# ShuoYangRobotics/Cerberus

Measured on NVIDIA H100. Metric: sliding-window solves/sec (10-frame x 150-feature windows), higher is better.
Workload: dtype f64

## Files before the change

cerberus_b200/csrc/cabi.cu:

```cuda
#include "../../include/cerberus_b200.h"
#include "solve_kernel.cuh"
#include "preint_kernel.cuh"
#include "feature_kernels.cuh"
#include "marg_kernels.cuh"
#include "pack_kernels.cuh"
#include "resident_kernels.cuh"
#include <string>
#include <vector>
#include <thread>
#include <cstring>
#include <cstdio>
#include <algorithm>
#include <chrono>
#include <cstdlib>
#include <cstdint>
#include <utility>

using namespace cerb;

static thread_local std::string g_err;
static int fail(int code, const std::string &msg) { g_err = msg; return code; }
#define CUDA_TRY(expr)                                                                                         \
    do {                                                                                                       \
        cudaError_t e_ = (expr);                                                                               \
        if (e_ != cudaSuccess) return fail(CERB_ERR_CUDA, std::string(#expr) + ": " + cudaGetErrorString(e_)); \
    } while (0)
#define COPY_TRY(h, dst, src, bytes, kind, s)                                                          \
    do {                                                                                               \
        (h)->traffic.count((kind), (bytes));                                                           \
        CUDA_TRY(cudaMemcpyAsync((dst), (src), (bytes), (kind), (s)));                                 \
    } while (0)
struct Traffic {
    int64_t h2d = 0, d2h = 0, ops = 0, staged = 0;
    void count(cudaMemcpyKind kind, size_t bytes) { if (kind == cudaMemcpyDeviceToDevice) return; (kind == cudaMemcpyHostToDevice ? h2d : d2h) += (int64_t)bytes; ops++; }
};

template <typename T> struct Resident {
    T *d = nullptr, *h = nullptr;
    size_t per = 0;
    T *at(size_t w) const { return d + w * per; }
    T *h_at(size_t w) const { return h + w * per; }
    size_t bytes(size_t n_windows) const { return n_windows * per * sizeof(T); }
};

struct CerbHandle {
    CerbSolverConfig cfg;
    int sm_count = 0, grid = 0;
    enum { MAX_CHUNKS = 32, LANES = 4 };
    cudaStream_t stream = nullptr, copy_stream = nullptr;
    cudaStream_t lane[LANES] = {};
    cudaEvent_t ev_lane[LANES] = {};
    cudaEvent_t ev_copy[MAX_CHUNKS] = {};
    cudaEvent_t ev0 = nullptr, ev1 = nullptr;
    bool ev_pending = false;
    double last_ms = 0; int last_launches = 0, last_dma_ops = 0; size_t last_staged_bytes = 0;
    int B = 0, F = 0, O = 0;
    int n = 0;
    Resident<CerbWindowDesc> rdesc; Resident<CerbFeature> rfeat; Resident<CerbObservation> robs; Resident<CerbWindowState> rstate;
    Resident<double> rpre, rlam;
    Resident<int> n_features, feat_start, feat_nobs, feat_off, flags, obs_stereo, prior_meta, rep_i, perm;
    Resident<double> obs, pre, sinfo, prior_J, prior_r, prior_x0, prior_Hp, state, state0, lam, lam0, rep_d;
    Resident<double> olam, ostate; Resident<CerbSolveReport> orep;
    double *d_ws = nullptr, *d_dbg = nullptr, *h_dbg = nullptr, *d_G = nullptr, *d_probe_repd = nullptr;
    int *d_probe_repi = nullptr;
    std::vector<void *> dev_bufs, host_bufs;
    std::vector<std::pair<uintptr_t, size_t>> regs;
    std::vector<int> nfeat, n0;
    int test_fail_factorizations = 0; double test_initial_mu = 0.0;
    bool solved = false;
    std::vector<int> h_perm; bool perm_valid = false;
    long ws_stride = 0;
    size_t smem_bytes = 0;
    std::vector<std::pair<char *, size_t>> arena; size_t arena_chunk = 0, arena_used = 0;
    Traffic traffic;
    int res_n = 0;
    Resident<int> pre_slot;
    std::vector<int> res_win;
    std::vector<int> res_extent;
    std::vector<char> res_prior_valid;
    std::vector<char> res_leg;
    Resident<double> step_J, step_r;
    bool prior_gathered = false;
    bool prior_gather_due = false;
    std::vector<unsigned char> res_mark;
};

static int create_impl(CerbHandle *h, const CerbSolverConfig *cfg, const cudaDeviceProp &prop);
#define CERB_DEVICE(h) do { if (h) { cudaError_t e_ = cudaSetDevice((h)->cfg.device); if (e_ != cudaSuccess) return fail(CERB_ERR_CUDA, std::string("cudaSetDevice: ") + cudaGetErrorString(e_)); } } while (0)

extern "C" {

const char *cerb_last_error(void) { return g_err.c_str(); }
const char *cerb_version(void) {
#if defined(CERB_CUSIM)
    return "cerberus_b200 0.1 (cusim test build)";
#else
    return "cerberus_b200 0.1 (sm_90a)";
#endif
}

void cerb_default_config(CerbSolverConfig *c) {
    std::memset(c, 0, sizeof(*c));
    c->device = 0; c->max_batch = 1024; c->max_features = 160; c->max_obs = 160 * CERB_NUM_FRAMES;
    c->max_num_iterations = 12; c->optimize_leg_bias = 1;
    c->g[0] = 0; c->g[1] = 0; c->g[2] = 9.805;
    c->visual_sqrt_info = 460.0 / 1.5; c->huber_delta = 1.0;
    c->initial_trust_region_radius = 1e4; c->max_trust_region_radius = 1e16; c->min_trust_region_radius = 1e-32;
    c->min_relative_decrease = 1e-3; c->function_tolerance = 1e-6; c->gradient_tolerance = 1e-10; c->parameter_tolerance = 1e-8;
}

void cerb_default_preint_config(CerbPreintConfig *p) {
    std::memset(p, 0, sizeof(*p));
    p->acc_n = 0.9; p->acc_n_z = 2.5; p->gyr_n = 0.05; p->acc_w = 0.0004; p->gyr_w = 0.0002;
    p->phi_n = 1e-5; p->dphi_n = 1e-5; p->rho_c_n = 1e-8; p->rho_nc_n = 1e-11;
    p->v_n_min_xy = 1e-3; p->v_n_min_z = 5e-3; p->v_n_min = 5e-3; p->v_n_max = 900.0;
    p->v_n_force_thres_ratio = 0.8; p->v_n_term1_steep = 10; p->v_n_term2_var_rescale = 1e-6; p->v_n_term3_distance_rescale = 1e-3;
    p->contact_sensor_type = 0;
    const double ox[4] = {0.1805, 0.1805, -0.1805, -0.1805}, oy[4] = {0.047, -0.047, 0.047, -0.047}, d[4] = {0.0838, -0.0838, 0.0838, -0.0838};
    for (int l = 0; l < 4; l++) { p->rho_fix[l][0] = ox[l]; p->rho_fix[l][1] = oy[l]; p->rho_fix[l][2] = d[l]; p->rho_fix[l][3] = 0.21; }
    p->R_br[0] = p->R_br[4] = p->R_br[8] = 1.0;
}


int cerb_create(const CerbSolverConfig *cfg, CerbHandle **out) {
    if (!cfg || !out) return fail(CERB_ERR_BAD_ARGUMENT, "cerb_create: null argument");
    if (cfg->max_batch < 1 || cfg->max_features < 1 || cfg->max_features > CERB_MAX_FEATURES || cfg->max_obs < 1)
        return fail(CERB_ERR_BAD_ARGUMENT, "cerb_create: bad capacities");
    int ndev = 0;
    if (cudaGetDeviceCount(&ndev) != cudaSuccess || ndev <= cfg->device)
        return fail(CERB_ERR_NO_DEVICE, "cerb_create: no CUDA device (this library has no CPU fallback)");
    CUDA_TRY(cudaSetDevice(cfg->device));
    cudaDeviceProp prop;
    CUDA_TRY(cudaGetDeviceProperties(&prop, cfg->device));
    CerbHandle *h = new CerbHandle();
    const int rc = create_impl(h, cfg, prop);
    if (rc != CERB_OK) { const std::string keep = g_err; cerb_destroy(h); g_err = keep; return rc; }
    *out = h;
    return CERB_OK;
}

}

template <typename T> static cudaError_t dmalloc(CerbHandle *h, T **p, size_t n) {
    const cudaError_t e = cudaMalloc((void **)p, n * sizeof(T));
    if (e == cudaSuccess) h->dev_bufs.push_back(*p);
    return e;
}
template <typename T> static cudaError_t hmalloc(CerbHandle *h, T **p, size_t n) {
    const cudaError_t e = cudaMallocHost((void **)p, n * sizeof(T));
    if (e == cudaSuccess) h->host_bufs.push_back(*p);
    return e;
}
template <typename T> static cudaError_t alloc(CerbHandle *h, Resident<T> &a, size_t per, bool mirror = false) {
    a.per = per;
    const cudaError_t e = dmalloc(h, &a.d, (size_t)h->B * per);
    return (e != cudaSuccess || !mirror) ? e : hmalloc(h, &a.h, (size_t)h->B * per);
}

static int create_impl(CerbHandle *h, const CerbSolverConfig *cfg, const cudaDeviceProp &prop) {
    h->cfg = *cfg; h->sm_count = prop.multiProcessorCount;
    if (const char *e = std::getenv("CERB_TEST_FAIL_FACTORIZATIONS")) h->test_fail_factorizations = std::atoi(e);
    if (const char *e = std::getenv("CERB_TEST_INITIAL_MU")) h->test_initial_mu = std::atof(e);
    h->B = cfg->max_batch; h->F = cfg->max_features; h->O = cfg->max_obs;
    h->grid = std::min(h->B, h->sm_count);
    h->smem_bytes = (size_t)SMEM_DOUBLES * sizeof(double);
    if (h->smem_bytes > prop.sharedMemPerBlockOptin) return fail(CERB_ERR_CUDA, "solve kernel needs more shared memory than the device offers");
    CUDA_TRY(cudaFuncSetAttribute(vilo_solve_kernel, cudaFuncAttributeMaxDynamicSharedMemorySize, (int)h->smem_bytes));
    CUDA_TRY(cudaFuncSetAttribute(prior_prepare_kernel, cudaFuncAttributeMaxDynamicSharedMemorySize, (int)(PRIOR_TROWS * PRIOR_TLD * sizeof(double))));
    CUDA_TRY(cudaStreamCreate(&h->stream));
    CUDA_TRY(cudaStreamCreate(&h->copy_stream));
    h->lane[0] = h->stream;
    for (int k = 1; k < CerbHandle::LANES; k++) CUDA_TRY(cudaStreamCreate(&h->lane[k]));
    for (int k = 0; k < CerbHandle::LANES; k++) CUDA_TRY(cudaEventCreate(&h->ev_lane[k]));
    for (int k = 0; k < CerbHandle::MAX_CHUNKS; k++) CUDA_TRY(cudaEventCreate(&h->ev_copy[k]));
    CUDA_TRY(cudaEventCreate(&h->ev0)); CUDA_TRY(cudaEventCreate(&h->ev1));
    const size_t F = h->F, O = h->O;
    h->ws_stride = ws_size(h->F);
    CUDA_TRY(alloc(h, h->rdesc, 1, true)); CUDA_TRY(alloc(h, h->rfeat, F, true)); CUDA_TRY(alloc(h, h->robs, O, true)); CUDA_TRY(alloc(h, h->rstate, 1, true));
    CUDA_TRY(alloc(h, h->rpre, CERB_WINDOW_SIZE * RAW_PRE_STRIDE, true)); CUDA_TRY(alloc(h, h->rlam, F, true)); CUDA_TRY(alloc(h, h->perm, F));
    CUDA_TRY(alloc(h, h->olam, F, true)); CUDA_TRY(alloc(h, h->ostate, ST_STRIDE, true)); CUDA_TRY(alloc(h, h->orep, 1, true));
    CUDA_TRY(alloc(h, h->n_features, 1)); CUDA_TRY(alloc(h, h->feat_start, F)); CUDA_TRY(alloc(h, h->feat_nobs, F)); CUDA_TRY(alloc(h, h->feat_off, F));
    CUDA_TRY(alloc(h, h->flags, 1)); CUDA_TRY(alloc(h, h->obs_stereo, O)); CUDA_TRY(alloc(h, h->prior_meta, PRIOR_META_STRIDE)); CUDA_TRY(alloc(h, h->rep_i, 4));
    CUDA_TRY(alloc(h, h->obs, NOBS_PLANES * O)); CUDA_TRY(alloc(h, h->pre, CERB_WINDOW_SIZE * PRE_STRIDE)); CUDA_TRY(alloc(h, h->sinfo, CERB_WINDOW_SIZE * 961));
    CUDA_TRY(alloc(h, h->prior_J, PRIOR_LD * PRIOR_LD, true)); CUDA_TRY(alloc(h, h->prior_r, PRIOR_LD, true)); CUDA_TRY(alloc(h, h->prior_x0, CERB_MAX_PRIOR_BLOCKS * 9));
    CUDA_TRY(alloc(h, h->prior_Hp, PRIOR_LD * PRIOR_LD));
    CUDA_TRY(alloc(h, h->state, ST_STRIDE)); CUDA_TRY(alloc(h, h->state0, ST_STRIDE)); CUDA_TRY(alloc(h, h->lam, F)); CUDA_TRY(alloc(h, h->lam0, F)); CUDA_TRY(alloc(h, h->rep_d, 2));
    CUDA_TRY(dmalloc(h, &h->d_ws, (size_t)CerbHandle::LANES * h->grid * h->ws_stride)); CUDA_TRY(dmalloc(h, &h->d_dbg, 2 * (NR + F) + 8)); CUDA_TRY(dmalloc(h, &h->d_G, 4));
    CUDA_TRY(dmalloc(h, &h->d_probe_repi, 4)); CUDA_TRY(dmalloc(h, &h->d_probe_repd, 2)); CUDA_TRY(hmalloc(h, &h->h_dbg, 2 * (NR + F) + 8));
    CUDA_TRY(alloc(h, h->pre_slot, CERB_WINDOW_SIZE + 1, true));
    h->nfeat.assign(h->B, 0); h->n0.assign(h->B, 0); h->res_extent.assign(h->B, 0); h->res_prior_valid.assign(h->B, 0); h->res_leg.assign(h->B, 1);
    CUDA_TRY(cudaMemcpy(h->d_G, cfg->g, 3 * sizeof(double), cudaMemcpyHostToDevice));
    return CERB_OK;
}

extern "C" {

void cerb_destroy(CerbHandle *h) {
    if (!h) return;
    cudaSetDevice(h->cfg.device);
    if (h->stream) cudaStreamSynchronize(h->stream);
    for (void *p : h->dev_bufs) cudaFree(p);
    for (auto &c : h->arena) cudaFree(c.first);
    for (auto &r : h->regs) cudaHostUnregister((void *)r.first);
    for (void *p : h->host_bufs) cudaFreeHost(p);
    if (h->ev0) cudaEventDestroy(h->ev0);
    if (h->ev1) cudaEventDestroy(h->ev1);
    for (int k = 0; k < CerbHandle::MAX_CHUNKS; k++) if (h->ev_copy[k]) cudaEventDestroy(h->ev_copy[k]);
    for (int k = 0; k < CerbHandle::LANES; k++) if (h->ev_lane[k]) cudaEventDestroy(h->ev_lane[k]);
    for (int k = 1; k < CerbHandle::LANES; k++) if (h->lane[k]) cudaStreamDestroy(h->lane[k]);
    if (h->copy_stream) cudaStreamDestroy(h->copy_stream);
    if (h->stream) cudaStreamDestroy(h->stream);
    delete h;
}

}
// ... 138 lines not shown
    plan_rows(h, pl, w0, cn, h->prior_J, 0, 1, 0,
              [&](int w) { return (const void *)descs[w].prior.linearized_jacobians; }, [&](int w) { return descs[w].prior.valid ? (size_t)descs[w].prior.n * descs[w].prior.n * 8 : (size_t)0; });
    plan_rows(h, pl, w0, cn, h->prior_r, 0, 1, 0,
              [&](int w) { return (const void *)descs[w].prior.linearized_residuals; }, [&](int w) { return descs[w].prior.valid ? (size_t)descs[w].prior.n * 8 : (size_t)0; });
    return run_plan(h, pl, s, t_stage_ms);
}

static int enqueue_pack(CerbHandle *h, int w0, int cn, cudaStream_t s) {
    PackParams P;
    P.n = cn; P.maxF = h->F; P.maxObs = h->O;
    P.rdesc = h->rdesc.at(w0); P.rfeat = h->rfeat.at(w0); P.robs = h->robs.at(w0); P.rpre = h->rpre.at(w0); P.rstate = h->rstate.at(w0); P.rlam = h->rlam.at(w0);
    P.n_features = h->n_features.at(w0); P.feat_start = h->feat_start.at(w0); P.feat_nobs = h->feat_nobs.at(w0); P.feat_off = h->feat_off.at(w0); P.flags = h->flags.at(w0);
    P.obs_stereo = h->obs_stereo.at(w0); P.prior_meta = h->prior_meta.at(w0); P.perm = h->perm.at(w0);
    P.obs = h->obs.at(w0); P.pre = h->pre.at(w0); P.prior_x0 = h->prior_x0.at(w0); P.state0 = h->state0.at(w0); P.lam0 = h->lam0.at(w0);
    if (h->res_n) { P.pre_slot = h->pre_slot.d; P.window = h->pre_slot.d + (size_t)cn * CERB_WINDOW_SIZE; }
    CERB_LAUNCH(pack_kernel, std::min(cn, 8 * h->sm_count), PACK_THREADS, 0, s, P);
    CUDA_TRY(cudaGetLastError());
    return CERB_OK;
}
static int upload(CerbHandle *h, int n, const CerbWindowDesc *descs, const CerbWindowState *states) {
    h->last_dma_ops = 0; h->last_staged_bytes = 0;
    int rc = upload_raw(h, 0, n, descs, states, h->stream, nullptr); if (rc) return rc;
    rc = enqueue_pack(h, 0, n, h->stream); if (rc) return rc;
    h->n = n; h->solved = false; h->perm_valid = false;
    return CERB_OK;
}
static int ensure_perm(CerbHandle *h) {
    if (h->perm_valid) return CERB_OK;
    h->h_perm.resize((size_t)h->B * h->perm.per);
    CUDA_TRY(cudaMemcpyAsync(h->h_perm.data(), h->perm.d, h->perm.bytes(h->n), cudaMemcpyDeviceToHost, h->stream));
    CUDA_TRY(cudaStreamSynchronize(h->stream));
    h->perm_valid = true;
    return CERB_OK;
}

static const Resident<double> &batch_prior_J(const CerbHandle *h) { return h->prior_gathered ? h->step_J : h->prior_J; }
static const Resident<double> &batch_prior_r(const CerbHandle *h) { return h->prior_gathered ? h->step_r : h->prior_r; }

static SolveParams make_params(CerbHandle *h, int w0, int n, int max_iters, double *dbg, int dbg_window) {
    SolveParams P;
    std::memset(&P, 0, sizeof(P));
    const CerbSolverConfig &c = h->cfg;
    P.n_windows = n; P.maxF = h->F; P.maxObs = h->O; P.max_iters = max_iters; P.optimize_leg_bias = c.optimize_leg_bias;
    for (int k = 0; k < 3; k++) P.G[k] = c.g[k];
    P.sqrt_info = c.visual_sqrt_info; P.huber = c.huber_delta;
    P.radius0 = c.initial_trust_region_radius; P.max_radius = c.max_trust_region_radius; P.min_radius = c.min_trust_region_radius;
    P.min_rel_dec = c.min_relative_decrease; P.ftol = c.function_tolerance; P.gtol = c.gradient_tolerance; P.ptol = c.parameter_tolerance;
    P.n_features = h->n_features.at(w0); P.feat_start = h->feat_start.at(w0); P.feat_nobs = h->feat_nobs.at(w0); P.feat_off = h->feat_off.at(w0); P.flags = h->flags.at(w0);
    P.obs = h->obs.at(w0); P.obs_stereo = h->obs_stereo.at(w0); P.pre = h->pre.at(w0); P.sinfo = h->sinfo.at(w0);
    P.prior_J = batch_prior_J(h).at(w0); P.prior_r = batch_prior_r(h).at(w0); P.prior_x0 = h->prior_x0.at(w0); P.prior_Hp = h->prior_Hp.at(w0); P.prior_meta = h->prior_meta.at(w0);
    P.state = h->state.at(w0); P.lam = h->lam.at(w0); P.rep_i = h->rep_i.at(w0); P.rep_d = h->rep_d.at(w0); P.ws = h->d_ws; P.ws_stride = h->ws_stride;
    P.dbg = dbg; P.dbg_window = dbg_window;
    P.test_fail_factorizations = h->test_fail_factorizations; P.test_initial_mu = h->test_initial_mu;
    P.no_bulk_copy = std::getenv("CERB_NO_TMA") != nullptr;
    return P;
}

static void enqueue_prepare(CerbHandle *h, int w0, int n, cudaStream_t s) {
    const int nfac = n * CERB_WINDOW_SIZE;
    CERB_LAUNCH(imu_leg_prepare_kernel, (nfac + 1) / 2, 64, 0, s, nfac, (const double *)h->pre.at(w0), h->sinfo.at(w0));
    CERB_LAUNCH(prior_prepare_kernel, n, 256, (size_t)PRIOR_TROWS * PRIOR_TLD * sizeof(double), s, (const double *)batch_prior_J(h).at(w0), (const int *)h->prior_meta.at(w0), h->prior_Hp.at(w0));
}

static int gather_priors(CerbHandle *h, cudaStream_t s) {
    if (!h->prior_gather_due) return CERB_OK;
    const int n = h->n;
    CERB_LAUNCH(prior_gather_kernel, std::min(n, 8 * h->sm_count), 256, 0, s, n, (const int *)(h->pre_slot.d + (size_t)n * CERB_WINDOW_SIZE), (const CerbWindowDesc *)h->rdesc.d,
                (const double *)h->prior_J.d, (const double *)h->prior_r.d, h->step_J.d, h->step_r.d);
    CUDA_TRY(cudaGetLastError());
    h->prior_gather_due = false;
    return CERB_OK;
}

static int enqueue_solve(CerbHandle *h, int w0, int n, int max_iters, double *dbg, int dbg_window, bool restore = true, bool probe = false, int lane = 0) {
    cudaStream_t s = h->lane[lane];
    if (restore) {
        CUDA_TRY(cudaMemcpyAsync(h->state.at(w0), h->state0.at(w0), h->state.bytes(n), cudaMemcpyDeviceToDevice, s));
        CUDA_TRY(cudaMemcpyAsync(h->lam.at(w0), h->lam0.at(w0), h->lam.bytes(n), cudaMemcpyDeviceToDevice, s));
    }
    int rc = gather_priors(h, s); if (rc) return rc;
    enqueue_prepare(h, w0, n, s);
    SolveParams P = make_params(h, w0, n, max_iters, dbg, dbg_window);
    P.ws = h->d_ws + (size_t)lane * h->grid * h->ws_stride;
    if (probe) { P.rep_i = h->d_probe_repi; P.rep_d = h->d_probe_repd; }
    if (max_iters > 0) h->solved = true;
    CERB_LAUNCH(vilo_solve_kernel, std::min(n, h->grid), SOLVE_THREADS, h->smem_bytes, s, P);
    CUDA_TRY(cudaGetLastError());
    return CERB_OK;
}
static int launch_solve(CerbHandle *h, int max_iters, double *dbg, int dbg_window, bool timed) {
    const int n = h->n;
    if (n < 1) return fail(CERB_ERR_BAD_ARGUMENT, "no resident batch");
    if (timed) CUDA_TRY(cudaEventRecord(h->ev0, h->stream));
    int rc = enqueue_solve(h, 0, n, max_iters, dbg, dbg_window); if (rc) return rc;
    if (timed) { CUDA_TRY(cudaEventRecord(h->ev1, h->stream)); h->ev_pending = true; h->last_launches = 3; }
    return CERB_OK;
}

static int collect_time(CerbHandle *h) {
    if (h->ev_pending) {
        CUDA_TRY(cudaEventSynchronize(h->ev1));
        float ms = 0; CUDA_TRY(cudaEventElapsedTime(&ms, h->ev0, h->ev1));
        h->last_ms = ms; h->ev_pending = false;
    }
    return CERB_OK;
}
// ... 712 lines not shown
```

cerberus_b200/csrc/solve_kernel.cuh:

```cuda
#pragma once
#include "eval_kernels.cuh"

namespace cerb {

#if defined(CERB_PHASE_TIMING) && !defined(CERB_CUSIM)
__device__ unsigned long long g_phase_cycles[48];
#define PH_DECL() long long ph_t = clock64()
#define PH_MARK_T(id, t) do { if ((threadIdx.x & 31) == 0) { const long long ph_n = clock64(); if (threadIdx.x == (t)) atomicAdd(&g_phase_cycles[id], (unsigned long long)(ph_n - ph_t)); ph_t = ph_n; } __syncwarp(); } while (0)
#define PH_MARK(id) PH_MARK_T(id, 0)
#define PH_ARG , long long &ph_t
#define PH_FWD , ph_t
#else
#define PH_DECL()
#define PH_MARK_T(id, t)
#define PH_MARK(id)
#define PH_ARG
#define PH_FWD
#endif

enum { CERB_WINDOW = 10, NX = 79, NYB = 13, NFR = 11, NY = 143, NR = 222, NRP = 224, HXX_SZ = 79 * 79, HXY_SZ = 79 * 143, X_TD = 78, SOLVE_THREADS = 256, FT = 64, TILE_LD = 33, NOBS_PLANES = 9 };
enum { HBLK = NYB * NYB, AD_SZ = NFR * HBLK, BO_SZ = (NFR - 1) * HBLK };
#ifndef CERB_SOLVE_MIN_BLOCKS
#define CERB_SOLVE_MIN_BLOCKS 1
#endif
enum { PIMG_HXY = HXX_SZ + 1, PIMG_REST = HXY_SZ + AD_SZ + BO_SZ, PIMG_SZ = PIMG_HXY + PIMG_REST, SMEM_HXX_PAD = 3 };
static_assert((PIMG_HXY * 8) % 16 == 0 && (PIMG_REST * 8) % 16 == 0 && ((HXX_SZ + SMEM_HXX_PAD) * 8) % 16 == 0, "bulk-copy alignment of the prior image");

struct SolveParams {
    int n_windows, maxF, maxObs, max_iters, optimize_leg_bias;
    double G[3], sqrt_info, huber;
    double radius0, max_radius, min_radius, min_rel_dec, ftol, gtol, ptol;
    const int *n_features, *feat_start, *feat_nobs, *feat_off, *flags;
    const double *obs; const int *obs_stereo;
    const double *pre;
    const double *sinfo;
    const double *prior_J, *prior_r, *prior_x0, *prior_Hp; const int *prior_meta;
    double *state, *lam;
    int *rep_i; double *rep_d;
    double *ws;
    long ws_stride;
    double *dbg; int dbg_window;
    double test_initial_mu;
    int no_bulk_copy;
    int test_fail_factorizations;
};

CERB_HD long ws_vecs(int F) { return (long)NX * F; }
CERB_HD long ws_prior(int F) { return (long)NX * F + 9L * F; }
CERB_HD long ws_chunks(int F) { return ws_prior(F) + PIMG_SZ; }
CERB_HD long ws_imuplan(int F) { return (ws_chunks(F) + (F + 4) / 2 + 8 + 1) & ~1L; }
CERB_HD long ws_size(int F) { return ws_imuplan(F) + 15 * 2 * 32 * 4 / 2 + 8; }
struct CtaWs {
    double *W, *hh, *gl, *sl, *Dl, *ghl, *gnl, *stl, *lamc, *sinv;
    int *chunks;
    int *imu_plan;
    double *pimg;
    int F;
};
CERB_D CtaWs ws_carve(const SolveParams &P) {
    double *ws = P.ws + (size_t)blockIdx.x * P.ws_stride;
    const int F = P.maxF;
    CtaWs v;
    v.W = ws;
    v.hh = ws + ws_vecs(F); v.gl = v.hh + F; v.sl = v.gl + F; v.Dl = v.sl + F; v.ghl = v.Dl + F; v.gnl = v.ghl + F; v.stl = v.gnl + F; v.lamc = v.stl + F; v.sinv = v.lamc + F;
    v.chunks = reinterpret_cast<int *>(ws + ws_chunks(F)); v.imu_plan = reinterpret_cast<int *>(ws + ws_imuplan(F));
    v.pimg = ws + ws_prior(F); v.F = F;
    return v;
}

struct Smem {
    double *Hxx, *Hxy, *Ad, *Bo;
    double *g, *sc, *D, *gh, *gn, *stp, *yv;
    double *xs, *xc;
    double *Rw, *Rex;
    double *Ju;
    double *lin;
    double *pdx, *pr;
    double *red;
    double *wj;
    double *sca;
    double *chain_col;
    double *idg;
    double *idx;
    int *ti;
    unsigned long long *mbar;
    double *tile;
};
enum { S_RADIUS = 0, S_MU, S_REUSE, S_XCOST, S_CCOST, S_ALPHA, S_GNORM2, S_GNNORM2, S_GDOTGN, S_MODEL, S_STEPNORM, S_XNORM, S_DLNORM,
       S_OK, S_DONE, S_TERM, S_ITER, S_NSUCC, S_INVALID, S_GMAX, S_INIT_COST, S_P, S_Q, S_VHV, S_LCOST, S_LNORM, S_LGMAX, S_COUNT };
static_assert(S_COUNT <= 32, "scalar slots overlap the chain's column line");
enum { TI_PRIOR_MAP = 0, TI_NCHUNKS = 96, TI_CHUNK_CACHE = 97, TI_CACHED_CHUNKS = 15, TI_CHAIN_DONE = 130, TI_IMU_MASK = 131, TI_INTS = 132 };
static_assert(TI_PRIOR_MAP + CERB_MAX_PRIOR_DIM <= TI_NCHUNKS && TI_CHUNK_CACHE + 2 * TI_CACHED_CHUNKS <= TI_CHAIN_DONE && TI_IMU_MASK < TI_INTS && TI_INTS % 2 == 0,
              "s.ti slots overlap");
enum { SMEM_DOUBLES = HXX_SZ + SMEM_HXX_PAD + HXY_SZ + AD_SZ + BO_SZ + 7 * NRP + 2 * ST_STRIDE + 99 + 18 + 3 + 31 * 39 + 960 + 192 + 8 * 256 + 128 * 8 + 32 + 32 + TI_INTS / 2 + 144 + 80 };

CERB_D void smem_carve(double *base, Smem &s) {
    double *p = base;
// ... 101 lines not shown
    if (g == 0) return c < 6 ? 6 * a + c : (c == 6 ? X_TD : -2);
    if (c >= 6) return -1;
    return g == 1 ? 6 * j + c : (g == 2 ? 66 + c : 72 + c);
}
CERB_D void vis_scatter(Smem &s, int ga, int gb, int ra, int rb, int a, int j, double v) {
    if (ga == gb && ra > rb) return;
    const int da = vis_col_dest(ga, ra, a, j), db = vis_col_dest(gb, rb, a, j);
    if (da == -1 || db == -1) return;
    if (da == -2) { if (db >= 0) s.g[db] += v; return; }
    if (db == -2) { s.g[da] += v; return; }
    if (da <= db) s.Hxx[da * NX + db] += v; else s.Hxx[db * NX + da] += v;
}
CERB_D void vis_jplan(const Smem &s, const double *smem_base, int el, int *base, int *ca, int *cj) {
    const int blk = el >> 6, ra = (el >> 3) & 7, rb = el & 7;
    const int hxx = (int)(s.Hxx - smem_base), g = (int)(s.g - smem_base);
    *base = -1; *ca = 0; *cj = 0;
    if (rb >= 6) return;
    if (blk == 0) {
        if (ra < 6) { *base = hxx + ra * NX + rb; *ca = 6 * NX; *cj = 6; }
        else if (ra == 6) { *base = hxx + rb * NX + X_TD; *cj = 6 * NX; }
        else { *base = g + rb; *cj = 6; }
    } else {
        if (ra >= 6 || (blk == 1 && ra > rb)) return;
        *base = hxx + ra * NX + (blk == 1 ? rb : (blk == 2 ? 66 + rb : 72 + rb)); *cj = 6 * NX + (blk == 1 ? 6 : 0);
    }
}
CERB_NOINLINE double vision_linearize(const SolveParams &P, int w, const double *x, const double *lam, double *W, double *hh, double *gl,
                                      const double *sl, bool prescale, const int *chunks, int tid) {
    CERB_DYN_SMEM(double, smem_base);
    Smem s; smem_carve(smem_base, s);
    const int nF = P.n_features[w], F = P.maxF, mo = P.maxObs;
    const double *obs = P.obs + (size_t)w * NOBS_PLANES * P.maxObs;
    const int *stereo = P.obs_stereo + (size_t)w * P.maxObs;
    double cost = 0.0;
    PH_DECL();
    for (int i = tid; i < NX * nF; i += SOLVE_THREADS) W[(i / nF) * F + (i % nF)] = 0.0;
    __syncthreads();
    const int wid = tid >> 5, lane = tid & 31;
    const int cam = tid >> 7, jj = (tid >> 6) & 1, fl = tid & 63;
    double *T = s.tile;
    double *jp = s.Ju;
    double *pp = (wid < 5) ? s.Ju + 8 * VJ_SZ + VP_SZ * wid : s.tile + VT_SZ + VP_SZ * (wid - 5);
    const int c8 = lane >> 2;
    const double *tq[4];
    bool tv[4];
    for (int g = 0; g < 4; g++) { const int pc = g == 0 ? c8 : 8 + 6 * (g - 1) + c8; tv[g] = (g == 0) || c8 < 6; tq[g] = T + (tv[g] ? pc : 0) * VT_LD + (lane & 3); }
    int jbase, jca, jcj;
    vis_jplan(s, smem_base, tid, &jbase, &jca, &jcj);
    const int nchunks = s.ti[TI_NCHUNKS];
    for (int ch = 0; ch < nchunks; ch++) {
        int c0, nc, a;
        if (ch < TI_CACHED_CHUNKS) { const int *cc = s.ti + TI_CHUNK_CACHE + 2 * ch; c0 = cc[0]; nc = cc[1] >> 8; a = cc[1] & 255; }
        else { c0 = chunks[1 + ch]; nc = chunks[2 + ch] - c0; a = P.feat_start[(size_t)w * F + c0]; }
        const int f = c0 + fl;
        const bool ev = fl < nc;
        int nobs = 0, off = 0;
        double lamf = 1.0, pix = 0.0, piy = 0.0, vix = 0.0, viy = 0.0, tdi = 0.0;
        const double slf = (prescale && ev) ? sl[f] : 1.0;
        if (ev) {
            nobs = P.feat_nobs[(size_t)w * F + f]; off = P.feat_off[(size_t)w * F + f];
            lamf = 1.0 / lam[f];
            pix = obs[0 * mo + off]; piy = obs[1 * mo + off]; vix = obs[2 * mo + off]; viy = obs[3 * mo + off]; tdi = obs[8 * mo + off];
        }
        ObsVals ov; ov.px = ov.py = ov.vx = ov.vy = ov.td = 0.0; ov.stereo = 0;
        { const int j = a + jj; if (ev && j < a + nobs) obs_fetch(obs, stereo, mo, off + (j - a), cam, ov); }
        for (int k = lane; k < VP_SZ; k += 32) pp[k] = 0.0;
        if (tid < 2 * (NFR - 1 - a)) {
            const int jq = a + 1 + (tid >> 1), cq = tid & 1;
            const m33 Rc = ldm33(cq ? s.Rex + 9 : s.Rex);
            const m33 A = mulT33(Rc, tr33(ldm33(s.Rw + 9 * jq)));
            const m33 ARi = mul33(A, ldm33(s.Rw + 9 * a));
            const m33 Tm = mul33(ARi, ldm33(s.Rex));
            double *C = s.lin + 27 * tid;
            for (int k = 0; k < 9; k++) { C[k] = A.m[k]; C[9 + k] = ARi.m[k]; C[18 + k] = Tm.m[k]; }
        } else if (tid == 32) {
            const m33 T3 = mul33(tr33(ldm33(s.Rex + 9)), ldm33(s.Rex));
            for (int k = 0; k < 9; k++) s.lin[540 + k] = T3.m[k];
        }
        __syncthreads();
        double h = 0.0, gq = 0.0, wT = 0.0, wI[6], wE0[6], wE1[6];
        for (int k = 0; k < 6; k++) { wI[k] = 0.0; wE0[k] = 0.0; wE1[k] = 0.0; }
        PH_MARK(20);
        for (int j0 = a; j0 < NFR; j0 += 2) {
            const int j = j0 + jj;
            bool valid = ev && j < a + nobs;
            int kind = PROJ_K1;
            if (valid) {
                if (j == a) { if (cam == 0 || !ov.stereo) valid = false; kind = PROJ_K3; }
                else if (cam == 1) { if (!ov.stereo) valid = false; kind = PROJ_K2; }
            }
            double wjv[6] = {0, 0, 0, 0, 0, 0};
            double *t0 = T + tid, *t1 = T + 256 + tid;
            if (valid) {
                const d3 tic = ld3(x + ST_EX), tc = kind == PROJ_K1 ? tic : ld3(x + ST_EX + 7);
                const double *Rcp = kind == PROJ_K1 ? s.Rex : s.Rex + 9;
                const double tdv = x[ST_TD];
                const d3 pts_i = mk3(pix, piy, 1.0), vel_i = mk3(vix, viy, 0.0);
                const d3 pts_i_td = pts_i - (tdv - tdi) * vel_i;
                const double pjx_td = ov.px - (tdv - ov.td) * ov.vx, pjy_td = ov.py - (tdv - ov.td) * ov.vy;
                const double inv_l = lamf;
                const d3 p_ci = inv_l * pts_i_td;
                const d3 p_bi = mv33(ldm33(s.Rex), p_ci) + tic;
                d3 p_bj = p_bi;
                if (kind != PROJ_K3) p_bj = mTv33(ldm33(s.Rw + 9 * j), (mv33(ldm33(s.Rw + 9 * a), p_bi) + ld3(x + ST_POSE + 7 * a)) - ld3(x + ST_POSE + 7 * j));
                const d3 p_cj = mTv33(ldm33(Rcp), p_bj - tc);
                const double iz = 1.0 / p_cj.z;
                double r0 = P.sqrt_info * (p_cj.x * iz - pjx_td), r1 = P.sqrt_info * (p_cj.y * iz - pjy_td);
                double cf; const double hw = huber_weight(P.huber, r0 * r0 + r1 * r1, &cf);
                cost += cf;
                r0 *= hw; r1 *= hw;
                const double q = hw * P.sqrt_info * iz, c0 = -q * p_cj.x * iz, c1 = -q * p_cj.y * iz;
                const d3 e0 = mk3(q, 0.0, c0), e1 = mk3(0.0, q, c1);
#define VIS_U(M, u0, u1) const d3 u0 = mk3(q * (M)[0] + c0 * (M)[6], q * (M)[1] + c0 * (M)[7], q * (M)[2] + c0 * (M)[8]), u1 = mk3(q * (M)[3] + c1 * (M)[6], q * (M)[4] + c1 * (M)[7], q * (M)[5] + c1 * (M)[8])
#define VIS_PUT(col, a0, a1) do { t0[(col) * VT_LD] = (a0); t1[(col) * VT_LD] = (a1); } while (0)
#define VIS_PUT3(col, v0_, v1_) do { VIS_PUT(col, (v0_).x, (v1_).x); VIS_PUT((col) + 1, (v0_).y, (v1_).y); VIS_PUT((col) + 2, (v0_).z, (v1_).z); } while (0)
                const double *Tm = kind == PROJ_K3 ? s.lin + 540 : s.lin + 27 * (2 * (j - a - 1) + cam) + 18;
                VIS_U(Tm, uT0, uT1);
                const d3 ptl = kind == PROJ_K3 ? pts_i : pts_i_td;
                const double l0 = -inv_l * inv_l * dot3(uT0, ptl), l1 = -inv_l * inv_l * dot3(uT1, ptl);
                const double d0 = -inv_l * dot3(uT0, vel_i) + hw * P.sqrt_info * ov.vx, d1 = -inv_l * dot3(uT1, vel_i) + hw * P.sqrt_info * ov.vy;
                h += l0 * l0 + l1 * l1; gq += l0 * r0 + l1 * r1; wT += d0 * l0 + d1 * l1;
                VIS_PUT(6, d0, d1); VIS_PUT(7, r0, r1);
                const d3 uC0 = mk3(q * Rcp[0] + c0 * Rcp[2], q * Rcp[3] + c0 * Rcp[5], q * Rcp[6] + c0 * Rcp[8]);
                const d3 uC1 = mk3(q * Rcp[1] + c1 * Rcp[2], q * Rcp[4] + c1 * Rcp[5], q * Rcp[7] + c1 * Rcp[8]);
                const d3 er0 = cross3(e0, p_cj), er1 = cross3(e1, p_cj);
                const d3 et0 = cross3(p_ci, uT0), et1 = cross3(p_ci, uT1);
                d3 E0t0, E0t1, E0r0, E0r1, E1t0, E1t1, E1r0, E1r1;
                if (kind == PROJ_K3) {
                    for (int k = 0; k < 6; k++) { VIS_PUT(k, 0.0, 0.0); VIS_PUT(8 + k, 0.0, 0.0); }
                    E0t0 = uC0; E0t1 = uC1; E0r0 = et0; E0r1 = et1; E1t0 = -uC0; E1t1 = -uC1; E1r0 = er0; E1r1 = er1;
                } else {
                    const double *C = s.lin + 27 * (2 * (j - a - 1) + cam);
                    VIS_U(C, uA0, uA1);
                    VIS_U(C + 9, uR0, uR1);
                    const d3 ir0 = cross3(p_bi, uR0), ir1 = cross3(p_bi, uR1);
                    const d3 jr0 = cross3(uC0, p_bj), jr1 = cross3(uC1, p_bj);
                    VIS_PUT3(0, uA0, uA1); VIS_PUT3(3, ir0, ir1);
                    VIS_PUT3(8, -uA0, -uA1); VIS_PUT3(11, jr0, jr1);
                    wI[0] += uA0.x * l0 + uA1.x * l1; wI[1] += uA0.y * l0 + uA1.y * l1; wI[2] += uA0.z * l0 + uA1.z * l1;
                    wI[3] += ir0.x * l0 + ir1.x * l1; wI[4] += ir0.y * l0 + ir1.y * l1; wI[5] += ir0.z * l0 + ir1.z * l1;
                    wjv[0] = -(uA0.x * l0 + uA1.x * l1); wjv[1] = -(uA0.y * l0 + uA1.y * l1); wjv[2] = -(uA0.z * l0 + uA1.z * l1);
                    wjv[3] = jr0.x * l0 + jr1.x * l1; wjv[4] = jr0.y * l0 + jr1.y * l1; wjv[5] = jr0.z * l0 + jr1.z * l1;
                    if (kind == PROJ_K1) {
                        E0t0 = uR0 - uC0; E0t1 = uR1 - uC1; E0r0 = et0 + er0; E0r1 = et1 + er1;
                        E1t0 = mk3(0, 0, 0); E1t1 = E1t0; E1r0 = E1t0; E1r1 = E1t0;
                    } else {
                        E0t0 = uR0; E0t1 = uR1; E0r0 = et0; E0r1 = et1; E1t0 = -uC0; E1t1 = -uC1; E1r0 = er0; E1r1 = er1;
                    }
                }
                VIS_PUT3(14, E0t0, E0t1); VIS_PUT3(17, E0r0, E0r1); VIS_PUT3(20, E1t0, E1t1); VIS_PUT3(23, E1r0, E1r1);
                wE0[0] += E0t0.x * l0 + E0t1.x * l1; wE0[1] += E0t0.y * l0 + E0t1.y * l1; wE0[2] += E0t0.z * l0 + E0t1.z * l1;
                wE0[3] += E0r0.x * l0 + E0r1.x * l1; wE0[4] += E0r0.y * l0 + E0r1.y * l1; wE0[5] += E0r0.z * l0 + E0r1.z * l1;
                wE1[0] += E1t0.x * l0 + E1t1.x * l1; wE1[1] += E1t0.y * l0 + E1t1.y * l1; wE1[2] += E1t0.z * l0 + E1t1.z * l1;
                wE1[3] += E1r0.x * l0 + E1r1.x * l1; wE1[4] += E1r0.y * l0 + E1r1.y * l1; wE1[5] += E1r0.z * l0 + E1r1.z * l1;
#undef VIS_U
#undef VIS_PUT
#undef VIS_PUT3
            } else {
                for (int k = 0; k < VT_COLS; k++) { t0[k * VT_LD] = 0.0; t1[k * VT_LD] = 0.0; }
            }
            const bool wrow = valid && j != a;
            if (wrow && cam == 0) for (int k = 0; k < 6; k++) W[(size_t)(6 * j + k) * F + f] = wjv[k] * (prescale ? s.sc[6 * j + k] * slf : 1.0);
            __syncthreads();
            PH_MARK(21);
            double wprev[6] = {0, 0, 0, 0, 0, 0};
            if (wrow && cam == 1) for (int k = 0; k < 6; k++) wprev[k] = W[(size_t)(6 * j + k) * F + f];
            { const int jn = j + 2; ov.stereo = 0; if (ev && jn < a + nobs) obs_fetch(obs, stereo, mo, off + (jn - a), cam, ov); }
            {
                const int jw = j0 + (wid >> 2), hw = (wid >> 1) & 1, par = wid & 1;
                const bool k3 = (jw == a);
                const int nkt = (nc + 3) >> 2;
                const bool work = jw < NFR && par < nkt;
                double acc[10][2];
                for (int k = 0; k < 10; k++) { acc[k][0] = 0.0; acc[k][1] = 0.0; }
                if (work) {
                    const int rb0 = 256 * hw + 64 * (wid >> 2) + 4 * par;
                    if (!k3) {
                        double v0 = tq[0][rb0], v1 = tv[1] ? tq[1][rb0] : 0.0, v2 = tv[2] ? tq[2][rb0] : 0.0;
                        for (int ks = par; ks < nkt; ks += 2) {
                            const int rn = rb0 + 4 * (ks + 2 - par);
                            const bool more = ks + 2 < nkt;
                            const double n0 = more ? tq[0][rn] : 0.0, n1 = (more && tv[1]) ? tq[1][rn] : 0.0, n2 = (more && tv[2]) ? tq[2][rn] : 0.0;
                            CERB_DMMA(acc[0][0], acc[0][1], v0, v0, acc[0][0], acc[0][1]);
                            CERB_DMMA(acc[1][0], acc[1][1], v0, v1, acc[1][0], acc[1][1]);
                            CERB_DMMA(acc[2][0], acc[2][1], v0, v2, acc[2][0], acc[2][1]);
                            CERB_DMMA(acc[4][0], acc[4][1], v1, v1, acc[4][0], acc[4][1]);
                            CERB_DMMA(acc[5][0], acc[5][1], v1, v2, acc[5][0], acc[5][1]);
                            CERB_DMMA(acc[7][0], acc[7][1], v2, v2, acc[7][0], acc[7][1]);
                            v0 = n0; v1 = n1; v2 = n2;
                        }
                    }
                    {
                        const int rb1 = rb0 + 128;
                        double v0 = tq[0][rb1], v1 = (!k3 && tv[1]) ? tq[1][rb1] : 0.0, v2 = tv[2] ? tq[2][rb1] : 0.0, v3 = tv[3] ? tq[3][rb1] : 0.0;
                        for (int ks = par; ks < nkt; ks += 2) {
                            const int rn = rb1 + 4 * (ks + 2 - par);
                            const bool more = ks + 2 < nkt;
                            const double n0 = more ? tq[0][rn] : 0.0, n1 = (more && !k3 && tv[1]) ? tq[1][rn] : 0.0, n2 = (more && tv[2]) ? tq[2][rn] : 0.0, n3 = (more && tv[3]) ? tq[3][rn] : 0.0;
                            CERB_DMMA(acc[0][0], acc[0][1], v0, v0, acc[0][0], acc[0][1]);
                            CERB_DMMA(acc[2][0], acc[2][1], v0, v2, acc[2][0], acc[2][1]);
                            CERB_DMMA(acc[3][0], acc[3][1], v0, v3, acc[3][0], acc[3][1]);
                            CERB_DMMA(acc[7][0], acc[7][1], v2, v2, acc[7][0], acc[7][1]);
                            CERB_DMMA(acc[8][0], acc[8][1], v2, v3, acc[8][0], acc[8][1]);
                            CERB_DMMA(acc[9][0], acc[9][1], v3, v3, acc[9][0], acc[9][1]);
                            if (!k3) {
                                CERB_DMMA(acc[1][0], acc[1][1], v0, v1, acc[1][0], acc[1][1]);
                                CERB_DMMA(acc[4][0], acc[4][1], v1, v1, acc[4][0], acc[4][1]);
                                CERB_DMMA(acc[5][0], acc[5][1], v1, v2, acc[5][0], acc[5][1]);
                                CERB_DMMA(acc[6][0], acc[6][1], v1, v3, acc[6][0], acc[6][1]);
                            }
                            v0 = n0; v1 = n1; v2 = n2; v3 = n3;
                        }
                    }
                    PH_MARK(28);
                    const int o = (lane >> 2) * 8 + 2 * (lane & 3);
                    pp[0 * 64 + o] += acc[0][0]; pp[0 * 64 + o + 1] += acc[0][1];
                    pp[1 * 64 + o] += acc[2][0]; pp[1 * 64 + o + 1] += acc[2][1];
                    pp[2 * 64 + o] += acc[3][0]; pp[2 * 64 + o + 1] += acc[3][1];
                    pp[3 * 64 + o] += acc[7][0]; pp[3 * 64 + o + 1] += acc[7][1];
                    pp[4 * 64 + o] += acc[8][0]; pp[4 * 64 + o + 1] += acc[8][1];
                    pp[5 * 64 + o] += acc[9][0]; pp[5 * 64 + o + 1] += acc[9][1];
                }
                {
                    const int o = wid * VJ_SZ + (lane >> 2) * 8 + 2 * (lane & 3);
                    jp[o] = acc[1][0]; jp[o + 1] = acc[1][1];
                    jp[64 + o] = acc[4][0]; jp[64 + o + 1] = acc[4][1];
                    jp[128 + o] = acc[5][0]; jp[128 + o + 1] = acc[5][1];
                    jp[192 + o] = acc[6][0]; jp[192 + o + 1] = acc[6][1];
                }
            }
            if (wrow && cam == 1) for (int k = 0; k < 6; k++) W[(size_t)(6 * j + k) * F + f] = wprev[k] + wjv[k] * (prescale ? s.sc[6 * j + k] * slf : 1.0);
            PH_MARK(29);
            __syncthreads();
            PH_MARK(22);
            if (jbase >= 0) {
                _Pragma("unroll")
                for (int fj = 0; fj < 2; fj++) {
                    const int jf = j0 + fj;
                    if (jf >= NFR || jf == a) continue;
                    const double *q = jp + (4 * fj) * VJ_SZ + tid;
                    smem_base[jbase + jca * a + jcj * jf] += ((q[0] + q[VJ_SZ]) + q[2 * VJ_SZ]) + q[3 * VJ_SZ];
                }
            }
            PH_MARK(23);
        }
        __syncthreads();
        {
            double *ex = T;
            ex[0 * 256 + tid] = h; ex[1 * 256 + tid] = gq; ex[2 * 256 + tid] = wT;
            for (int k = 0; k < 6; k++) { ex[(3 + k) * 256 + tid] = wI[k]; ex[(9 + k) * 256 + tid] = wE0[k]; ex[(15 + k) * 256 + tid] = wE1[k]; }
        }
        __syncthreads();
        for (int e = tid; e < VP_SZ; e += SOLVE_THREADS) {
            double v = 0.0;
            for (int wq = 0; wq < 8; wq++) v += ((wq < 5) ? s.Ju + 8 * VJ_SZ + VP_SZ * wq : s.tile + VT_SZ + VP_SZ * (wq - 5))[e];
            const int blk = e >> 6, ra = (e >> 3) & 7, rb = e & 7;
            const int ga = blk < 3 ? 0 : (blk < 5 ? 2 : 3), gb = blk == 0 ? 0 : (blk == 1 || blk == 3 ? 2 : 3);
            vis_scatter(s, ga, gb, ra, rb, a, a, v);
        }
        if (tid < 64 && ev) {
            const double *ex = T;
            double q[21];
            for (int k = 0; k < 21; k++) q[k] = ((ex[k * 256 + tid] + ex[k * 256 + 64 + tid]) + ex[k * 256 + 128 + tid]) + ex[k * 256 + 192 + tid];
            hh[f] = q[0] * slf * slf; gl[f] = q[1] * slf;
            W[(size_t)X_TD * F + f] = q[2] * (prescale ? s.sc[X_TD] * slf : 1.0);
            for (int k = 0; k < 6; k++) {
                W[(size_t)(6 * a + k) * F + f] = q[3 + k] * (prescale ? s.sc[6 * a + k] * slf : 1.0);
                W[(size_t)(66 + k) * F + f] = q[9 + k] * (prescale ? s.sc[66 + k] * slf : 1.0);
                W[(size_t)(72 + k) * F + f] = q[15 + k] * (prescale ? s.sc[72 + k] * slf : 1.0);
            }
        }
        __syncthreads();
        PH_MARK(24);
    }
    return cost;
}

CERB_D void imu_lin_all(const SolveParams &P, Smem &s, int w, const double *x, bool want_jac, int tid) {
    if (tid < CERB_WINDOW) {
        const double *pre = P.pre + ((size_t)w * CERB_WINDOW + tid) * PRE_STRIDE;
        IMULegLin *L = reinterpret_cast<IMULegLin *>(s.lin + 96 * tid);
        imu_leg_linearize(pre, x + ST_POSE + 7 * tid, x + ST_SB + 9 * tid, x + ST_LB + 4 * tid, x + ST_POSE + 7 * (tid + 1),
                          x + ST_SB + 9 * (tid + 1), x + ST_LB + 4 * (tid + 1), P.G, want_jac, L);
    }
    __syncthreads();
}

CERB_D double prior_residual(const SolveParams &P, Smem &s, int w, const double *x, int tid) {
    const int *meta = P.prior_meta + (size_t)w * PRIOR_META_STRIDE;
    if (!meta[0]) return 0.0;
    const int n = meta[1], nb = meta[2];
    const double *J = P.prior_J + (size_t)w * PRIOR_LD * PRIOR_LD, *r0 = P.prior_r + (size_t)w * PRIOR_LD, *x0 = P.prior_x0 + (size_t)w * 16 * 9;
    if (tid < nb) {
        const int kind = meta[4 + 3 * tid], index = meta[5 + 3 * tid], col = meta[6 + 3 * tid];
        prior_block_dx(kind, x + prior_block_state_offset(kind, index), x0 + 9 * tid, s.pdx + col);
    }
    __syncthreads();
    int parts = SOLVE_THREADS / n; if (parts > 4) parts = 4; if (parts < 1) parts = 1;
    const int kc = (n + parts - 1) / parts;
    double *part = s.red;
    for (int e = tid; e < parts * n; e += SOLVE_THREADS) {
        const int p = e / n, i = e % n;
        const int k1 = (p + 1) * kc < n ? (p + 1) * kc : n;
        double t = 0.0;
        for (int k = p * kc; k < k1; k++) t += J[(size_t)k * n + i] * s.pdx[k];
        part[p * PRIOR_LD + i] = t;
    }
    __syncthreads();
    double cost = 0.0;
    for (int i = tid; i < n; i += SOLVE_THREADS) {
        double t = r0[i];
        for (int p = 0; p < parts; p++) t += part[p * PRIOR_LD + i];
        s.pr[i] = t; cost += 0.5 * t * t;
// ... 1181 lines not shown
```

Baseline: 34820.

## Process four frames per pass for small feature chunks in visual linearization

When a feature chunk holds at most 32 features, threads with lane index 32 and above now handle frames offset by two. Each outer-loop pass therefore covers four observing frames instead of two, which roughly halves the number of passes and barriers for small chunks. The upper-half partial sums (cost, Hessian, gradient, W rows) are exchanged through shared memory and folded into the lower half, and the DMMA block reductions run twice per pass. The cost is extra syncthreads, added shared-memory traffic, and register pressure from keeping the acc array live outside its block. An environment flag restores the old two-frame path.

```diff
diff --git a/cerberus_b200/csrc/cabi.cu b/cerberus_b200/csrc/cabi.cu
--- a/cerberus_b200/csrc/cabi.cu
+++ b/cerberus_b200/csrc/cabi.cu
@@ -67,6 +67,7 @@
     std::vector<std::pair<uintptr_t, size_t>> regs;
     std::vector<int> nfeat, n0;
     int test_fail_factorizations = 0; double test_initial_mu = 0.0;
+    int test_two_frame_passes = 0;
     bool solved = false;
     std::vector<int> h_perm; bool perm_valid = false;
     long ws_stride = 0;
@@ -161,6 +162,7 @@
     h->cfg = *cfg; h->sm_count = prop.multiProcessorCount;
     if (const char *e = std::getenv("CERB_TEST_FAIL_FACTORIZATIONS")) h->test_fail_factorizations = std::atoi(e);
     if (const char *e = std::getenv("CERB_TEST_INITIAL_MU")) h->test_initial_mu = std::atof(e);
+    if (const char *e = std::getenv("CERB_TEST_TWO_FRAME_PASSES")) h->test_two_frame_passes = std::atoi(e) != 0;
     h->B = cfg->max_batch; h->F = cfg->max_features; h->O = cfg->max_obs;
     h->grid = std::min(h->B, h->sm_count);
     h->smem_bytes = (size_t)SMEM_DOUBLES * sizeof(double);
@@ -405,6 +407,7 @@
     P.state = h->state.at(w0); P.lam = h->lam.at(w0); P.rep_i = h->rep_i.at(w0); P.rep_d = h->rep_d.at(w0); P.ws = h->d_ws; P.ws_stride = h->ws_stride;
     P.dbg = dbg; P.dbg_window = dbg_window;
     P.test_fail_factorizations = h->test_fail_factorizations; P.test_initial_mu = h->test_initial_mu;
+    P.test_two_frame_passes = h->test_two_frame_passes;
     P.no_bulk_copy = std::getenv("CERB_NO_TMA") != nullptr;
     return P;
 }
diff --git a/cerberus_b200/csrc/solve_kernel.cuh b/cerberus_b200/csrc/solve_kernel.cuh
--- a/cerberus_b200/csrc/solve_kernel.cuh
+++ b/cerberus_b200/csrc/solve_kernel.cuh
@@ -43,6 +43,7 @@
     double test_initial_mu;
     int no_bulk_copy;
     int test_fail_factorizations;
+    int test_two_frame_passes;
 };
 
 CERB_HD long ws_vecs(int F) { return (long)NX * F; }
@@ -250,8 +251,11 @@
         int c0, nc, a;
         if (ch < TI_CACHED_CHUNKS) { const int *cc = s.ti + TI_CHUNK_CACHE + 2 * ch; c0 = cc[0]; nc = cc[1] >> 8; a = cc[1] & 255; }
         else { c0 = chunks[1 + ch]; nc = chunks[2 + ch] - c0; a = P.feat_start[(size_t)w * F + c0]; }
-        const int f = c0 + fl;
-        const bool ev = fl < nc;
+        const int fp = (nc <= 32 && !P.test_two_frame_passes) ? 4 : 2;
+        const bool up = fp == 4 && fl >= 32;
+        const int fe = up ? fl - 32 : fl, jo = up ? 2 : 0;
+        const int f = c0 + fe;
+        const bool ev = fe < nc;
         int nobs = 0, off = 0;
         double lamf = 1.0, pix = 0.0, piy = 0.0, vix = 0.0, viy = 0.0, tdi = 0.0;
         const double slf = (prescale && ev) ? sl[f] : 1.0;
@@ -261,7 +265,7 @@
             pix = obs[0 * mo + off]; piy = obs[1 * mo + off]; vix = obs[2 * mo + off]; viy = obs[3 * mo + off]; tdi = obs[8 * mo + off];
         }
         ObsVals ov; ov.px = ov.py = ov.vx = ov.vy = ov.td = 0.0; ov.stereo = 0;
-        { const int j = a + jj; if (ev && j < a + nobs) obs_fetch(obs, stereo, mo, off + (j - a), cam, ov); }
+        { const int j = a + jj + jo; if (ev && j < a + nobs) obs_fetch(obs, stereo, mo, off + (j - a), cam, ov); }
         for (int k = lane; k < VP_SZ; k += 32) pp[k] = 0.0;
         if (tid < 2 * (NFR - 1 - a)) {
             const int jq = a + 1 + (tid >> 1), cq = tid & 1;
@@ -278,9 +282,11 @@
         __syncthreads();
         double h = 0.0, gq = 0.0, wT = 0.0, wI[6], wE0[6], wE1[6];
         for (int k = 0; k < 6; k++) { wI[k] = 0.0; wE0[k] = 0.0; wE1[k] = 0.0; }
+        double *cfu = s.Ju + 8 * VJ_SZ + 5 * VP_SZ + (tid >> 6) * 32 + (tid & 31);
+        if (up) *cfu = 0.0;
         PH_MARK(20);
-        for (int j0 = a; j0 < NFR; j0 += 2) {
-            const int j = j0 + jj;
+        for (int j0 = a; j0 < NFR; j0 += fp) {
+            const int j = j0 + jj + jo;
             bool valid = ev && j < a + nobs;
             int kind = PROJ_K1;
             if (valid) {
@@ -305,7 +311,7 @@
                 const double iz = 1.0 / p_cj.z;
                 double r0 = P.sqrt_info * (p_cj.x * iz - pjx_td), r1 = P.sqrt_info * (p_cj.y * iz - pjy_td);
                 double cf; const double hw = huber_weight(P.huber, r0 * r0 + r1 * r1, &cf);
-                cost += cf;
+                if (up) *cfu = cf; else cost += cf;
                 r0 *= hw; r1 *= hw;
                 const double q = hw * P.sqrt_info * iz, c0 = -q * p_cj.x * iz, c1 = -q * p_cj.y * iz;
                 const d3 e0 = mk3(q, 0.0, c0), e1 = mk3(0.0, q, c1);
@@ -363,82 +369,111 @@
             PH_MARK(21);
             double wprev[6] = {0, 0, 0, 0, 0, 0};
             if (wrow && cam == 1) for (int k = 0; k < 6; k++) wprev[k] = W[(size_t)(6 * j + k) * F + f];
-            { const int jn = j + 2; ov.stereo = 0; if (ev && jn < a + nobs) obs_fetch(obs, stereo, mo, off + (jn - a), cam, ov); }
+            { const int jn = j + fp; ov.stereo = 0; if (ev && jn < a + nobs) obs_fetch(obs, stereo, mo, off + (jn - a), cam, ov); }
+            double acc[10][2];
             {
-                const int jw = j0 + (wid >> 2), hw = (wid >> 1) & 1, par = wid & 1;
-                const bool k3 = (jw == a);
+                const int hw = (wid >> 1) & 1, par = wid & 1;
                 const int nkt = (nc + 3) >> 2;
-                const bool work = jw < NFR && par < nkt;
-                double acc[10][2];
-                for (int k = 0; k < 10; k++) { acc[k][0] = 0.0; acc[k][1] = 0.0; }
-                if (work) {
-                    const int rb0 = 256 * hw + 64 * (wid >> 2) + 4 * par;
-                    if (!k3) {
-                        double v0 = tq[0][rb0], v1 = tv[1] ? tq[1][rb0] : 0.0, v2 = tv[2] ? tq[2][rb0] : 0.0;
-                        for (int ks = par; ks < nkt; ks += 2) {
-                            const int rn = rb0 + 4 * (ks + 2 - par);
-                            const bool more = ks + 2 < nkt;
-                            const double n0 = more ? tq[0][rn] : 0.0, n1 = (more && tv[1]) ? tq[1][rn] : 0.0, n2 = (more && tv[2]) ? tq[2][rn] : 0.0;
-                            CERB_DMMA(acc[0][0], acc[0][1], v0, v0, acc[0][0], acc[0][1]);
-                            CERB_DMMA(acc[1][0], acc[1][1], v0, v1, acc[1][0], acc[1][1]);
-                            CERB_DMMA(acc[2][0], acc[2][1], v0, v2, acc[2][0], acc[2][1]);
-                            CERB_DMMA(acc[4][0], acc[4][1], v1, v1, acc[4][0], acc[4][1]);
-                            CERB_DMMA(acc[5][0], acc[5][1], v1, v2, acc[5][0], acc[5][1]);
-                            CERB_DMMA(acc[7][0], acc[7][1], v2, v2, acc[7][0], acc[7][1]);
-                            v0 = n0; v1 = n1; v2 = n2;
-                        }
-                    }
-                    {
-                        const int rb1 = rb0 + 128;
-                        double v0 = tq[0][rb1], v1 = (!k3 && tv[1]) ? tq[1][rb1] : 0.0, v2 = tv[2] ? tq[2][rb1] : 0.0, v3 = tv[3] ? tq[3][rb1] : 0.0;
-                        for (int ks = par; ks < nkt; ks += 2) {
-                            const int rn = rb1 + 4 * (ks + 2 - par);
-                            const bool more = ks + 2 < nkt;
-                            const double n0 = more ? tq[0][rn] : 0.0, n1 = (more && !k3 && tv[1]) ? tq[1][rn] : 0.0, n2 = (more && tv[2]) ? tq[2][rn] : 0.0, n3 = (more && tv[3]) ? tq[3][rn] : 0.0;
-                            CERB_DMMA(acc[0][0], acc[0][1], v0, v0, acc[0][0], acc[0][1]);
-                            CERB_DMMA(acc[2][0], acc[2][1], v0, v2, acc[2][0], acc[2][1]);
-                            CERB_DMMA(acc[3][0], acc[3][1], v0, v3, acc[3][0], acc[3][1]);
-                            CERB_DMMA(acc[7][0], acc[7][1], v2, v2, acc[7][0], acc[7][1]);
-                            CERB_DMMA(acc[8][0], acc[8][1], v2, v3, acc[8][0], acc[8][1]);
-                            CERB_DMMA(acc[9][0], acc[9][1], v3, v3, acc[9][0], acc[9][1]);
-                            if (!k3) {
+                _Pragma("unroll 1")
+                for (int u = 0; u < fp / 2; u++) {
+                    const int jw = j0 + (wid >> 2) + 2 * u;
+                    const bool k3 = (jw == a);
+                    const bool work = jw < NFR && par < nkt;
+                    for (int k = 0; k < 10; k++) { acc[k][0] = 0.0; acc[k][1] = 0.0; }
+                    if (work) {
+                        const int rb0 = 256 * hw + 64 * (wid >> 2) + 32 * u + 4 * par;
+                        if (!k3) {
+                            double v0 = tq[0][rb0], v1 = tv[1] ? tq[1][rb0] : 0.0, v2 = tv[2] ? tq[2][rb0] : 0.0;
+                            for (int ks = par; ks < nkt; ks += 2) {
+                                const int rn = rb0 + 4 * (ks + 2 - par);
+                                const bool more = ks + 2 < nkt;
+                                const double n0 = more ? tq[0][rn] : 0.0, n1 = (more && tv[1]) ? tq[1][rn] : 0.0, n2 = (more && tv[2]) ? tq[2][rn] : 0.0;
+                                CERB_DMMA(acc[0][0], acc[0][1], v0, v0, acc[0][0], acc[0][1]);
                                 CERB_DMMA(acc[1][0], acc[1][1], v0, v1, acc[1][0], acc[1][1]);
+                                CERB_DMMA(acc[2][0], acc[2][1], v0, v2, acc[2][0], acc[2][1]);
                                 CERB_DMMA(acc[4][0], acc[4][1], v1, v1, acc[4][0], acc[4][1]);
                                 CERB_DMMA(acc[5][0], acc[5][1], v1, v2, acc[5][0], acc[5][1]);
-                                CERB_DMMA(acc[6][0], acc[6][1], v1, v3, acc[6][0], acc[6][1]);
+                                CERB_DMMA(acc[7][0], acc[7][1], v2, v2, acc[7][0], acc[7][1]);
+                                v0 = n0; v1 = n1; v2 = n2;
                             }
-                            v0 = n0; v1 = n1; v2 = n2; v3 = n3;
                         }
+                        {
+                            const int rb1 = rb0 + 128;
+                            double v0 = tq[0][rb1], v1 = (!k3 && tv[1]) ? tq[1][rb1] : 0.0, v2 = tv[2] ? tq[2][rb1] : 0.0, v3 = tv[3] ? tq[3][rb1] : 0.0;
+                            for (int ks = par; ks < nkt; ks += 2) {
+                                const int rn = rb1 + 4 * (ks + 2 - par);
+                                const bool more = ks + 2 < nkt;
+                                const double n0 = more ? tq[0][rn] : 0.0, n1 = (more && !k3 && tv[1]) ? tq[1][rn] : 0.0, n2 = (more && tv[2]) ? tq[2][rn] : 0.0, n3 = (more && tv[3]) ? tq[3][rn] : 0.0;
+                                CERB_DMMA(acc[0][0], acc[0][1], v0, v0, acc[0][0], acc[0][1]);
+                                CERB_DMMA(acc[2][0], acc[2][1], v0, v2, acc[2][0], acc[2][1]);
+                                CERB_DMMA(acc[3][0], acc[3][1], v0, v3, acc[3][0], acc[3][1]);
+                                CERB_DMMA(acc[7][0], acc[7][1], v2, v2, acc[7][0], acc[7][1]);
+                                CERB_DMMA(acc[8][0], acc[8][1], v2, v3, acc[8][0], acc[8][1]);
+                                CERB_DMMA(acc[9][0], acc[9][1], v3, v3, acc[9][0], acc[9][1]);
+                                if (!k3) {
+                                    CERB_DMMA(acc[1][0], acc[1][1], v0, v1, acc[1][0], acc[1][1]);
+                                    CERB_DMMA(acc[4][0], acc[4][1], v1, v1, acc[4][0], acc[4][1]);
+                                    CERB_DMMA(acc[5][0], acc[5][1], v1, v2, acc[5][0], acc[5][1]);
+                                    CERB_DMMA(acc[6][0], acc[6][1], v1, v3, acc[6][0], acc[6][1]);
+                                }
+                                v0 = n0; v1 = n1; v2 = n2; v3 = n3;
+                            }
+                        }
+                        PH_MARK(28);
+                        const int o = (lane >> 2) * 8 + 2 * (lane & 3);
+                        pp[0 * 64 + o] += acc[0][0]; pp[0 * 64 + o + 1] += acc[0][1];
+                        pp[1 * 64 + o] += acc[2][0]; pp[1 * 64 + o + 1] += acc[2][1];
+                        pp[2 * 64 + o] += acc[3][0]; pp[2 * 64 + o + 1] += acc[3][1];
+                        pp[3 * 64 + o] += acc[7][0]; pp[3 * 64 + o + 1] += acc[7][1];
+                        pp[4 * 64 + o] += acc[8][0]; pp[4 * 64 + o + 1] += acc[8][1];
+                        pp[5 * 64 + o] += acc[9][0]; pp[5 * 64 + o + 1] += acc[9][1];
                     }
-                    PH_MARK(28);
-                    const int o = (lane >> 2) * 8 + 2 * (lane & 3);
-                    pp[0 * 64 + o] += acc[0][0]; pp[0 * 64 + o + 1] += acc[0][1];
-                    pp[1 * 64 + o] += acc[2][0]; pp[1 * 64 + o + 1] += acc[2][1];
-                    pp[2 * 64 + o] += acc[3][0]; pp[2 * 64 + o + 1] += acc[3][1];
-                    pp[3 * 64 + o] += acc[7][0]; pp[3 * 64 + o + 1] += acc[7][1];
-                    pp[4 * 64 + o] += acc[8][0]; pp[4 * 64 + o + 1] += acc[8][1];
-                    pp[5 * 64 + o] += acc[9][0]; pp[5 * 64 + o + 1] += acc[9][1];
-                }
-                {
-                    const int o = wid * VJ_SZ + (lane >> 2) * 8 + 2 * (lane & 3);
-                    jp[o] = acc[1][0]; jp[o + 1] = acc[1][1];
-                    jp[64 + o] = acc[4][0]; jp[64 + o + 1] = acc[4][1];
-                    jp[128 + o] = acc[5][0]; jp[128 + o + 1] = acc[5][1];
-                    jp[192 + o] = acc[6][0]; jp[192 + o + 1] = acc[6][1];
+                    if (u == 0) {
+                        const int o = wid * VJ_SZ + (lane >> 2) * 8 + 2 * (lane & 3);
+                        jp[o] = acc[1][0]; jp[o + 1] = acc[1][1];
+                        jp[64 + o] = acc[4][0]; jp[64 + o + 1] = acc[4][1];
+                        jp[128 + o] = acc[5][0]; jp[128 + o + 1] = acc[5][1];
+                        jp[192 + o] = acc[6][0]; jp[192 + o + 1] = acc[6][1];
+                    }
                 }
             }
             if (wrow && cam == 1) for (int k = 0; k < 6; k++) W[(size_t)(6 * j + k) * F + f] = wprev[k] + wjv[k] * (prescale ? s.sc[6 * j + k] * slf : 1.0);
             PH_MARK(29);
             __syncthreads();
             PH_MARK(22);
-            if (jbase >= 0) {
+            const auto scatter_frames = [&](const double *src, int jf0) {
+                if (jbase < 0) return;
                 _Pragma("unroll")
                 for (int fj = 0; fj < 2; fj++) {
-                    const int jf = j0 + fj;
+                    const int jf = jf0 + fj;
                     if (jf >= NFR || jf == a) continue;
-                    const double *q = jp + (4 * fj) * VJ_SZ + tid;
+                    const double *q = src + (4 * fj) * VJ_SZ + tid;
                     smem_base[jbase + jca * a + jcj * jf] += ((q[0] + q[VJ_SZ]) + q[2 * VJ_SZ]) + q[3 * VJ_SZ];
                 }
+            };
+            double *jq = T, *hv = T + 8 * VJ_SZ;
+            if (fp == 4) {
+                const int o = wid * VJ_SZ + (lane >> 2) * 8 + 2 * (lane & 3);
+                jq[o] = acc[1][0]; jq[o + 1] = acc[1][1]; jq[64 + o] = acc[4][0]; jq[64 + o + 1] = acc[4][1];
+                jq[128 + o] = acc[5][0]; jq[128 + o + 1] = acc[5][1]; jq[192 + o] = acc[6][0]; jq[192 + o + 1] = acc[6][1];
+                if (up) {
+                    double *v = hv + (tid - 32);
+                    v[0] = *cfu; v[256] = h; v[2 * 256] = gq; v[3 * 256] = wT;
+                    for (int k = 0; k < 6; k++) { v[(4 + k) * 256] = wI[k]; v[(10 + k) * 256] = wE0[k]; v[(16 + k) * 256] = wE1[k]; }
+                    *cfu = 0.0; h = 0.0; gq = 0.0; wT = 0.0;
+                    for (int k = 0; k < 6; k++) { wI[k] = 0.0; wE0[k] = 0.0; wE1[k] = 0.0; }
+                }
+            }
+            scatter_frames(jp, j0);
+            if (fp == 4) {
+                __syncthreads();
+                scatter_frames(jq, j0 + 2);
+                if (!up) {
+                    const double *v = hv + tid;
+                    cost += v[0]; h += v[256]; gq += v[2 * 256]; wT += v[3 * 256];
+                    for (int k = 0; k < 6; k++) { wI[k] += v[(4 + k) * 256]; wE0[k] += v[(10 + k) * 256]; wE1[k] += v[(16 + k) * 256]; }
+                }
+                __syncthreads();
             }
             PH_MARK(23);
         }
@@ -456,7 +491,7 @@
             const int ga = blk < 3 ? 0 : (blk < 5 ? 2 : 3), gb = blk == 0 ? 0 : (blk == 1 || blk == 3 ? 2 : 3);
             vis_scatter(s, ga, gb, ra, rb, a, a, v);
         }
-        if (tid < 64 && ev) {
+        if (tid < 64 && ev && !up) {
             const double *ex = T;
             double q[21];
             for (int k = 0; k < 21; k++) q[k] = ((ex[k * 256 + tid] + ex[k * 256 + 64 + tid]) + ex[k * 256 + 128 + tid]) + ex[k * 256 + 192 + tid];
```

Result: no change. 35080 (median of 6 runs) (+0.8%).
